# nz0001na/MorphGANformer

Measured on AMD Instinct MI355X. Metric: latent-projection iters/sec @1024^2, k=17 latents, higher is better.
Workload: dtype f32; 1 GPU; configs[1]: single 1024x1024 face per GPU, Wing+LPIPS(squeeze)+MSE literal-mode projection step, noise_mode=random, seeded synthetic weights/targets/landmarks; k=17, z_dim=32, targets_per_gpu=1, parallelism=pair-sharded x1, graph_replay=True, loss_generator_overlap=True, steps_per_forward=32

## Files before the change

include/mgf.h:

```cpp
#ifndef MGF_H_
#define MGF_H_

#include <stdint.h>

#ifdef __cplusplus
extern "C" {
#endif

typedef void* mgf_stream_t;

enum { MGF_OK = 0, MGF_EINVAL = -1, MGF_EUNSUPPORTED = -2, MGF_ELAUNCH = -3, MGF_ETOOBIG = -4 };
enum { MGF_F32 = 0, MGF_F64 = 1, MGF_F16 = 2 };
enum { MGF_FILTER_SEPARABLE = 2 };
enum { MGF_FILTER_LARGE = 4 };
enum { MGF_ACT_LINEAR = 1, MGF_ACT_RELU = 2, MGF_ACT_LRELU = 3, MGF_ACT_TANH = 4, MGF_ACT_SIGMOID = 5,
       MGF_ACT_ELU = 6, MGF_ACT_SELU = 7, MGF_ACT_SOFTPLUS = 8, MGF_ACT_SWISH = 9,
       MGF_ACT_RELU_POST = 10 };

const char* mgf_last_error(void);
int mgf_version(void);
int mgf_device_ok(void);

int mgf_bias_act(void* y, const void* x, const void* b, const void* xref, const void* yref, const void* dy,
                 int dtype, int64_t numel, int64_t step_b, int64_t size_b,
// ... 79 lines not shown
int mgf_conv1x1_force_shape(int32_t channel_blocks);

int mgf_conv3x3s2_few_inputs_f32(float* y, const float* x, const float* w, const float* bias, int32_t n, int32_t cin, int32_t in_h,
                                 int32_t in_w, int32_t cout, int32_t relu, mgf_stream_t stream);
int mgf_tconv3x3s2_few_outputs_f32(float* y, const float* x, const float* wp, int32_t n, int32_t cin, int32_t h, int32_t w, int32_t cout,
                                   int32_t cout_pad, int32_t pitch, int64_t y_plane, int64_t y_batch, mgf_stream_t stream);
int mgf_conv3x3_winograd3_up2res_f32(float* y, const float* x, const float* u, const float* in_scale, const float* out_scale,
                                     const float* residual_low, int32_t n, int32_t cin, int32_t h, int32_t w, int32_t cout,
                                     int32_t out_scale_stride, const mgf_epilogue* ep, mgf_stream_t stream);
int mgf_winograd3_force_shape(int32_t shape);
int mgf_conv3x3_winograd3_rgb_f32(float* rgb_out, const float* x, const float* u, const float* in_scale, const float* out_scale,
                                  const float* rgb_w, const float* rgb_bias, int32_t n, int32_t cin, int32_t h, int32_t w, int32_t cout,
                                  int32_t out_scale_stride, int32_t rgb_channels, mgf_stream_t stream);
int mgf_conv3x3_winograd_f32(float* y, const float* x, const float* u, const float* in_scale, const float* out_scale, int32_t n,
                             int32_t cin, int32_t h, int32_t w, int32_t cout, int32_t out_scale_stride, const mgf_epilogue* ep,
                             mgf_stream_t stream);

int mgf_tconv3x3s2_border_f32(float* t, const float* x, const float* wp, const float* in_scale, const float* out_scale, int32_t n,
                              int32_t cin, int32_t h, int32_t w, int32_t cout, int32_t cout_pad, int64_t t_pitch, int64_t t_plane,
                              int64_t t_batch, int64_t out_scale_stride, mgf_stream_t stream);

int mgf_tconv3x3s2_blur_f32(float* y, const float* x, const float* wp, const float* in_scale, const float* out_scale, const float* f1d,
                            float gain, int32_t n, int32_t cin, int32_t h, int32_t w, int32_t cout, int32_t cout_pad, int64_t y_pitch,
                            int64_t y_plane, int64_t y_batch, int64_t out_scale_stride, const mgf_epilogue* ep, mgf_stream_t stream);

int mgf_tconv3x3s2_winograd_f32(float* t, const float* x, const float* u, const float* in_scale, const float* out_scale, int32_t n,
                                int32_t cin, int32_t h, int32_t w, int32_t cout, int32_t pitch, int64_t t_plane, int64_t t_batch,
                                int64_t out_scale_stride, mgf_stream_t stream);
int mgf_tconv_winograd_weights_f32(float* u, const float* w, int32_t cout, int32_t cin, double gain, mgf_stream_t stream);

int mgf_pack_conv_weights(float* wp, float* wsq, const float* w, int32_t cout, int32_t cin, int32_t kh, int32_t kw,
                          int32_t cout_pad, float gain, int32_t flip, mgf_stream_t stream);

typedef struct mgf_style_job {
    const float* aff_w;
    const float* aff_b;
    const float* wsq;
    float* s;
    float* d;
    int32_t cin, cout;
    int32_t w_offset;
    float aff_gain, style_gain;
} mgf_style_job;
int mgf_demod_f32(float* d, const float* s, const float* wsq, int32_t n, int32_t cin, int32_t cout, mgf_stream_t stream);
int mgf_demod_bwd_f32(float* ds, const float* dd, const float* d, const float* s, const float* wsq, int32_t n, int32_t cin, int32_t cout,
                      mgf_stream_t stream);
int mgf_style_demod(const mgf_style_job* job, const float* ws, int64_t ws_stride_n, int32_t n, int32_t wdim, mgf_stream_t stream);
int mgf_style_demod_multi(const mgf_style_job* jobs_dev, int32_t njobs, const float* ws, int64_t ws_stride_n,
                          int32_t n, int32_t wdim, int32_t max_cin, mgf_stream_t stream);

int mgf_duplex_attention(float* y, const float* x, const float* wqc, const float* spos, const float* vwb,
                         int32_t n, int32_t c, int32_t f, int32_t t,
                         const mgf_epilogue* ep, int32_t ep_w, float* probs, int32_t* argmax, mgf_stream_t stream);

int mgf_att_map_upsample_f32(float* out, const float* probs, int32_t n, int32_t side, int32_t t, int32_t out_res, int32_t layer,
                             int32_t n_layers, mgf_stream_t stream);

typedef struct mgf_attn_job {
    const float* wmv;
    const float* bmv;
    float* vwb;
    int32_t c;
    int32_t w_offset;
} mgf_attn_job;
int mgf_attn_values(const mgf_attn_job* job, const float* ws, int64_t ws_stride_n, int64_t ws_stride_t, int32_t n, int32_t t,
                    int32_t wdim, mgf_stream_t stream);
int mgf_attn_values_multi(const mgf_attn_job* jobs_dev, int32_t njobs, const float* ws, int64_t ws_stride_n, int64_t ws_stride_t,
                          int32_t n, int32_t t, int32_t wdim, mgf_stream_t stream);

int mgf_randn_f32(float* out, int64_t n, uint64_t seed, void* state, mgf_stream_t stream);
int mgf_rgb_weights_f32(float* out, const float* w, const float* s, int32_t n, int32_t c, int32_t cout, mgf_stream_t stream);
int mgf_randn_keyed_f32(float* out, const int32_t* sides, int32_t n_layers, int32_t n, const uint64_t* key, const int32_t* step,
                        int32_t step_stride, int32_t step_add, int32_t step_max, int32_t aux0, int32_t aux_add, mgf_stream_t stream);
int mgf_torgb_compose_weights_f32(float* w_eff, const float* w_last, const float* s_last, const float* d_last, const float* w_rgb,
                                  const float* s_rgb, int32_t n, int32_t cin, int32_t cout, int32_t rgb_channels, mgf_stream_t stream);
int mgf_conv3x3_few_outputs_f32(float* y, const float* x, const float* w, const float* bias, int32_t n, int32_t cin, int32_t h, int32_t wd,
                                int32_t cout, mgf_stream_t stream);

int64_t mgf_mapping_param_floats(int32_t k, int32_t dim, int32_t n_res_layers);
int mgf_mapping_forward(float* w, const float* z, const float* params, int32_t n, int32_t k, int32_t dim,
                        int32_t n_res_layers, int32_t normalize_global, mgf_stream_t stream);

int64_t mgf_reduce_scratch_floats(void);
int mgf_mse_f32(float* out, const float* a, const float* b, int32_t n, int64_t numel, int64_t b_batch_stride, float scale,
                int32_t accumulate, float* scratch, mgf_stream_t stream);
int64_t mgf_dssim_scratch_bytes(int32_t n, int32_t c, int32_t h, int32_t w);
int mgf_dssim_u8_f32(float* out, const float* img, const float* target, int32_t n, int32_t c, int32_t h, int32_t w, int64_t t_batch_stride,
                     float data_range, float scale, int32_t accumulate, void* scratch, mgf_stream_t stream);
int mgf_dssim_f32(float* out, const float* img, const float* target, int32_t n, int32_t c, int32_t h, int32_t w, int64_t t_batch_stride,
                  float data_range, float scale, int32_t accumulate, void* scratch, mgf_stream_t stream);
int mgf_dssim_grad_f32(float* dimg, float* out, const float* img, const float* target, int32_t n, int32_t c, int32_t h, int32_t w,
                       int64_t t_batch_stride, float data_range, float scale, int32_t accumulate_dimg, int32_t accumulate_out, void* scratch,
                       mgf_stream_t stream);
int64_t mgf_msssim_scratch_bytes(int32_t n, int32_t c, int32_t h, int32_t w, int32_t levels);
int mgf_msssim_f32(float* out, const float* img, const float* target, int32_t n, int32_t c, int32_t h, int32_t w, int64_t t_batch_stride,
                   const double* weights, int32_t levels, float data_range, float scale, int32_t accumulate, void* scratch, mgf_stream_t stream);
int mgf_msssim_grad_f32(float* dimg, float* out, const float* img, const float* target, int32_t n, int32_t c, int32_t h, int32_t w,
                        int64_t t_batch_stride, const double* weights, int32_t levels, float data_range, float scale, int32_t accumulate_dimg,
                        int32_t accumulate_out, void* scratch, mgf_stream_t stream);
int64_t mgf_lbp_scratch_bytes(int32_t n);
int mgf_lbp_gray224_u8(uint8_t* gray, const float* img, const int32_t* tables, int32_t n, int32_t h, int32_t w, int32_t true_rgb_order,
                       mgf_stream_t stream);
int mgf_lbp_codes_u8(uint8_t* codes, const uint8_t* gray, const double* offsets, int32_t n, mgf_stream_t stream);
int mgf_lbp_distance_f64(double* out, const uint8_t* gray, const uint8_t* target_codes, const double* offsets, int32_t n, void* scratch,
                         mgf_stream_t stream);
int mgf_wing_loss_f64(double* out, const double* pred, const double* target, int32_t n, int64_t numel, double omega, double epsilon,
// ... 240 lines not shown
```

morphganformer_amd/csrc/attention.hip:

```cpp
#include "mgf_common.h"

namespace {

typedef float v2f __attribute__((ext_vector_type(2)));
__device__ __forceinline__ void att_fma_row(v2f (&s2)[8], float xv, const float4* w4) {
    const v2f x2 = {xv, xv};
#pragma unroll
    for (int q = 0; q < 4; ++q) {
        const float4 w = w4[q];
        const v2f lo = {w.x, w.y}, hi = {w.z, w.w};
        s2[2 * q] += x2 * lo;
        s2[2 * q + 1] += x2 * hi;
    }
}
__device__ __forceinline__ float att_dot_row(const v2f (&s2)[8], const float4* w4) {
    v2f g2 = {0.f, 0.f};
#pragma unroll
    for (int q = 0; q < 4; ++q) {
        const float4 w = w4[q];
        const v2f lo = {w.x, w.y}, hi = {w.z, w.w};
        g2 += s2[2 * q] * lo;
        g2 += s2[2 * q + 1] * hi;
    }
    return g2.x + g2.y;
}

constexpr int TMAX = 16;
constexpr int UNR = 4;

struct AttnParams {
    float* y;
    const float* x;
    const float* wqc;
    const float* spos;
    const float* vwb;
    int n, c, f, t;
    int c_pad;
    mgf_epilogue ep;
    int has_ep;
    float* probs;
    int32_t* argmax;
};

template <int PXB, int NCH>
__global__ __launch_bounds__(256) void duplex_attention_kernel(AttnParams p) {
    constexpr int G = 256 / PXB;
    extern __shared__ float lds[];
    float* tab = lds;
    float* part = lds + (size_t)p.c_pad * TMAX;
    const int tid = threadIdx.x;
    const int px = tid % PXB, grp = tid / PXB;
    const int n = blockIdx.y;
    const int f0 = blockIdx.x * PXB;
    const int f = f0 + px;
    const bool valid = f < p.f;
    const int fc = valid ? f : p.f - 1;
    const float* xn = p.x + (int64_t)n * p.c * p.f;
    const int T = p.t;

    float xreg[NCH > 0 ? NCH : 1];
    if (NCH > 0) {
#pragma unroll
        for (int k = 0; k < NCH; ++k) {
            const int c = (k / UNR) * G * UNR + grp * UNR + (k % UNR);
            xreg[k] = xn[(int64_t)c * p.f + fc];
        }
    }

    auto stage_table = [&](const float* src) {
        if (T == TMAX) {
            const int n4 = p.c * (TMAX / 4), n4_pad = p.c_pad * (TMAX / 4);
            const float4* s4 = reinterpret_cast<const float4*>(src);
            float4* d4 = reinterpret_cast<float4*>(tab);
            for (int i0 = tid; i0 < n4_pad; i0 += 256 * 4) {
                float4 v[4];
#pragma unroll
                for (int u = 0; u < 4; ++u) {
                    const int i = i0 + 256 * u;
                    v[u] = i < n4 ? s4[i] : make_float4(0.f, 0.f, 0.f, 0.f);
                }
#pragma unroll
                for (int u = 0; u < 4; ++u) {
                    const int i = i0 + 256 * u;
                    if (i < n4_pad) d4[i] = v[u];
                }
            }
        } else {
            for (int i = tid; i < p.c_pad * TMAX; i += 256) {
                const int c = i / TMAX, t = i % TMAX;
                tab[i] = (c < p.c && t < T) ? src[(int64_t)c * T + t] : 0.f;
            }
        }
    };
    stage_table(p.wqc);
// ... 333 lines not shown
            for (int g = 0; g < G; ++g) v += part[(g * (TMAX + 1) + t) * PXB + px];
            fin[t * PXB + px] = v;
        }
        __syncthreads();
        float m = -3.0e38f;
#pragma unroll
        for (int t = 0; t < TMAX; ++t) {
            const float v = fin[t * PXB + px] + spk[t];
            m = fmaxf(m, v);
            s[t] = v;
        }
        sq = fin[TMAX * PXB + px];
        float den = 0.f;
        int best = 0;
        float bestv = -3.0e38f;
#pragma unroll
        for (int t = 0; t < TMAX; ++t) {
            if (s[t] > bestv) { bestv = s[t]; best = t; }
            s[t] = __expf(s[t] - m);
            den += s[t];
        }
        const float inv = 1.f / den;
        const float rs = rsqrtf(sq / (float)p.c + 1e-8f);
#pragma unroll
        for (int t = 0; t < TMAX; ++t) s[t] *= inv;
        if (grp == 0 && valid) {
            if (p.probs)
                for (int t = 0; t < TMAX; ++t) p.probs[((int64_t)n * p.f + f) * TMAX + t] = s[t];
            if (p.argmax) p.argmax[(int64_t)n * p.f + f] = best;
        }
#pragma unroll
        for (int q = 0; q < TMAX / 2; ++q) s2[q] = v2f{s[2 * q] * rs, s[2 * q + 1] * rs};

        float* yn = p.y + (int64_t)n * p.c * p.f;
#pragma unroll
        for (int k = 0; k < NCH; ++k) {
            const int c = (k / UNR) * G * UNR + grp * UNR + (k % UNR);
            const float g = att_dot_row(s2, reinterpret_cast<const float4*>(tabv + c * TMAX));
            float v = xk[k] * g;
            if (p.has_ep) {
                v += nzk;
                if (p.ep.bias) v += p.ep.bias[c];
                if (p.ep.act == MGF_ACT_LRELU) v = v > 0.f ? v : v * p.ep.alpha;
                else if (p.ep.act == MGF_ACT_RELU) v = v > 0.f ? v : 0.f;
                v *= p.ep.gain;
                v += rk[k];
            }
            if (valid) yn[(int64_t)c * p.f + f] = v;
        }
    }
}

typedef float f32x16 __attribute__((ext_vector_type(16)));
template <int NW>
__global__ __launch_bounds__(NW * 64, NW == 4 ? 4 : 2) void duplex_attention_mfma_kernel(AttnParams p) {
    __shared__ float red[NW][9][64];
    const int tid = threadIdx.x, lane = tid & 63;
    const int wv = __builtin_amdgcn_readfirstlane(tid >> 6);
    const int l31 = lane & 31, half = lane >> 5;
    const int n = blockIdx.y, f0 = blockIdx.x * 32;
    const int cw0 = wv * 64;
    const int64_t nb = (int64_t)n * p.c * p.f;
    const bool ep = p.has_ep != 0;
    const __amdgpu_buffer_rsrc_t rx = __builtin_amdgcn_make_buffer_rsrc((void*)(p.x + nb), 0, p.c * p.f * 4, 0x00020000);
    const float* resp = (ep && p.ep.residual) ? p.ep.residual + nb : nullptr;
    const __amdgpu_buffer_rsrc_t rres = __builtin_amdgcn_make_buffer_rsrc((void*)(resp ? resp : p.x), 0, resp ? p.c * p.f * 4 : 0, 0x00020000);
    const __amdgpu_buffer_rsrc_t rq = __builtin_amdgcn_make_buffer_rsrc((void*)p.wqc, 0, p.c * TMAX * 4, 0x00020000);
    const __amdgpu_buffer_rsrc_t rv = __builtin_amdgcn_make_buffer_rsrc((void*)(p.vwb + (int64_t)n * p.c * TMAX), 0, p.c * TMAX * 4, 0x00020000);
    const __amdgpu_buffer_rsrc_t rsp = __builtin_amdgcn_make_buffer_rsrc((void*)p.spos, 0, p.f * TMAX * 4, 0x00020000);
    const float* biasp = (ep && p.ep.bias) ? p.ep.bias : nullptr;
    const __amdgpu_buffer_rsrc_t rb = __builtin_amdgcn_make_buffer_rsrc((void*)(biasp ? biasp : p.x), 0, biasp ? p.c * 4 : 0, 0x00020000);
    auto rowof = [](int r) { return (r & 3) + 8 * (r >> 2); };

    const unsigned xo = (unsigned)((cw0 + 4 * half) * p.f + f0 + l31) * 4u;
    const unsigned qo = l31 < TMAX ? (unsigned)((cw0 + 4 * half) * TMAX + l31) * 4u : 0xFFFFFFF0u;
    float xr[2][16], a1[2][16];
#pragma unroll
    for (int cb = 0; cb < 2; ++cb)
#pragma unroll
        for (int r = 0; r < 16; ++r) {
            const int ch = 32 * cb + rowof(r);
            xr[cb][r] = __builtin_bit_cast(float, __builtin_amdgcn_raw_buffer_load_b32(rx, xo, ch * p.f * 4, 0));
            a1[cb][r] = __builtin_bit_cast(float, __builtin_amdgcn_raw_buffer_load_b32(rq, qo, ch * TMAX * 4, 0));
        }
    float sp[8];
#pragma unroll
    for (int r = 0; r < 8; ++r)
        sp[r] = __builtin_bit_cast(float, __builtin_amdgcn_raw_buffer_load_b32(rsp, (unsigned)((f0 + l31) * TMAX + 4 * half) * 4u, rowof(r) * 4, 0));
    float nz = 0.f;
    if (ep && p.ep.noise) nz = p.ep.noise[(int64_t)(p.ep.noise_n > 1 ? n : 0) * p.f + f0 + l31] * (p.ep.noise_strength ? *p.ep.noise_strength : 1.f);

    f32x16 acc;
#pragma unroll
    for (int r = 0; r < 16; ++r) acc[r] = 0.f;
    float sq = 0.f;
#pragma unroll
    for (int cb = 0; cb < 2; ++cb)
#pragma unroll
        for (int r = 0; r < 16; ++r) {
            acc = __builtin_amdgcn_mfma_f32_32x32x2f32(a1[cb][r], xr[cb][r], acc, 0, 0, 0);
            sq += xr[cb][r] * xr[cb][r];
        }
    float rr[2][16];
#pragma unroll
    for (int cb = 0; cb < 2; ++cb)
#pragma unroll
        for (int r = 0; r < 16; ++r)
            rr[cb][r] = __builtin_bit_cast(float, __builtin_amdgcn_raw_buffer_load_b32(rres, xo, (32 * cb + rowof(r)) * p.f * 4, 0));
#pragma unroll
    for (int r = 0; r < 8; ++r) red[wv][r][lane] = acc[r];
    red[wv][8][lane] = sq;
    __syncthreads();
    float s[8];
#pragma unroll
    for (int r = 0; r < 8; ++r) {
        float v = sp[r];
#pragma unroll
        for (int w = 0; w < NW; ++w) v += red[w][r][lane];
        s[r] = v;
    }
    sq = 0.f;
#pragma unroll
    for (int w = 0; w < NW; ++w) sq += red[w][8][lane];
    sq += __shfl_xor(sq, 32, 64);
    float m = s[0];
    int best = 4 * half;
#pragma unroll
    for (int r = 1; r < 8; ++r) {
        if (s[r] > m) { m = s[r]; best = rowof(r) + 4 * half; }
    }
    {
        const float om = __shfl_xor(m, 32, 64);
        const int ob = __shfl_xor(best, 32, 64);
        if (om > m || (om == m && ob < best)) { m = om; best = ob; }
    }
    float den = 0.f;
#pragma unroll
    for (int r = 0; r < 8; ++r) { s[r] = __expf(s[r] - m); den += s[r]; }
    den += __shfl_xor(den, 32, 64);
    const float inv = 1.f / den;
    const float rs = rsqrtf(sq / (float)p.c + 1e-8f);
    if (wv == 0) {
        if (p.probs) {
#pragma unroll
            for (int r = 0; r < 8; ++r) p.probs[((int64_t)n * p.f + f0 + l31) * TMAX + rowof(r) + 4 * half] = s[r] * inv;
        }
        if (p.argmax && half == 0) p.argmax[(int64_t)n * p.f + f0 + l31] = best;
    }
    const float ps = inv * rs;
#pragma unroll
    for (int r = 0; r < 8; ++r) s[r] *= ps;

    float* yn = p.y + nb;
    const float slope = !ep ? 1.f : (p.ep.act == MGF_ACT_LRELU ? p.ep.alpha : (p.ep.act == MGF_ACT_RELU ? 0.f : 1.f));
    const float gain = ep ? p.ep.gain : 1.f;
#pragma unroll
    for (int cb = 0; cb < 2; ++cb) {
        const unsigned vo = (unsigned)((cw0 + 32 * cb + l31) * TMAX + 4 * half) * 4u;
        const float4 va = __builtin_bit_cast(float4, __builtin_amdgcn_raw_buffer_load_b128(rv, vo, 0, 0));
        const float4 vb = __builtin_bit_cast(float4, __builtin_amdgcn_raw_buffer_load_b128(rv, vo + 32u, 0, 0));
        float bv[16];
#pragma unroll
        for (int r = 0; r < 16; ++r)
            bv[r] = __builtin_bit_cast(float, __builtin_amdgcn_raw_buffer_load_b32(rb, (unsigned)(cw0 + 32 * cb + 4 * half) * 4u, rowof(r) * 4, 0));
        const float a2[8] = {va.x, va.y, va.z, va.w, vb.x, vb.y, vb.z, vb.w};
        f32x16 g;
#pragma unroll
        for (int r = 0; r < 16; ++r) g[r] = 0.f;
#pragma unroll
        for (int j = 0; j < 8; ++j) g = __builtin_amdgcn_mfma_f32_32x32x2f32(a2[j], s[j], g, 0, 0, 0);
#pragma unroll
        for (int r = 0; r < 16; ++r) {
            float v = xr[cb][r] * g[r];
            v += nz;
            v += bv[r];
            v = v > 0.f ? v : v * slope;
            v = v * gain + rr[cb][r];
            yn[(int64_t)(cw0 + 32 * cb + rowof(r) + 4 * half) * p.f + f0 + l31] = v;
        }
    }
}

__global__ __launch_bounds__(256) void att_map_upsample_kernel(float* out, const float* probs, int t, int s, int R, int layer, int layers,
                                                               int64_t total) {
    const int f = R / s;
    for (int64_t i = (int64_t)blockIdx.x * 256 + threadIdx.x; i < total; i += (int64_t)gridDim.x * 256) {
        const int x = (int)(i % R);
        int64_t r = i / R;
        const int y = (int)(r % R);
        r /= R;
        const int tt = (int)(r % t);
        const int64_t n = r / t;
        out[(((n * t + tt) * layers + layer) * R + y) * (int64_t)R + x] = probs[(n * s * s + (int64_t)(y / f) * s + x / f) * t + tt];
    }
}

template <int PXB>
void launch_attention(const AttnParams& p, size_t lds, hipStream_t st) {
    constexpr int G = 256 / PXB;
    const int nch = (p.c % (G * UNR) == 0) ? p.c / G : 0;
    if (p.t == TMAX && (nch == 16 || nch == 32 || nch == 64) && (nch * G) % 64 == 0) {
        const size_t lds_r = ((size_t)p.c * TMAX + (size_t)(G + 1) * (TMAX + 1) * PXB) * sizeof(float);
        static const char* nb_env = mgf_knob("MGF_ATTN_NBLK");
        constexpr int NBLK = 4;
        if (PXB == 16 && nch == 16 && p.f >= 4096 && p.f % (PXB * NBLK) == 0 && !(nb_env && nb_env[0] == '1')) {
            const size_t lds_2 = ((size_t)2 * p.c * TMAX + (size_t)(G + 1) * (TMAX + 1) * PXB) * sizeof(float);
            hipLaunchKernelGGL((duplex_attention_blocks_kernel<PXB, 16, NBLK>), dim3((unsigned)(p.f / (PXB * NBLK)), p.n), dim3(256), lds_2, st, p);
            return;
        }
        const dim3 grid((unsigned)mgf_cdiv(p.f, PXB), p.n);
        if (nch == 16) hipLaunchKernelGGL((duplex_attention_reg_kernel<PXB, 16>), grid, dim3(256), lds_r, st, p);
        else if (nch == 32) hipLaunchKernelGGL((duplex_attention_reg_kernel<PXB, 32>), grid, dim3(256), lds_r, st, p);
        else hipLaunchKernelGGL((duplex_attention_reg_kernel<PXB, 64>), grid, dim3(256), lds_r, st, p);
        return;
    }
    const dim3 grid((unsigned)mgf_cdiv(p.f, PXB), p.n);
    hipLaunchKernelGGL((duplex_attention_kernel<PXB, 0>), grid, dim3(256), lds, st, p);
}

}

extern "C" int mgf_duplex_attention(float* y, const float* x, const float* wqc, const float* spos, const float* vwb, int32_t n,
                                    int32_t c, int32_t f, int32_t t, const mgf_epilogue* ep, int32_t ep_w, float* probs,
                                    int32_t* argmax, mgf_stream_t stream) {
    (void)ep_w;
    MGF_REQUIRE(y && x && wqc && spos && vwb, MGF_EINVAL, "duplex_attention: null pointer");
    MGF_REQUIRE(n >= 1 && c >= 1 && f >= 1, MGF_EINVAL, "duplex_attention: bad shape");
    MGF_REQUIRE(t >= 1 && t <= TMAX, MGF_EUNSUPPORTED, "duplex_attention: supports 1..%d latent components (got %d)", TMAX, t);
    MGF_REQUIRE(n <= 65535 && (int64_t)n * c * f <= INT32_MAX, MGF_ETOOBIG, "duplex_attention: tensor too large");
    if (ep) MGF_REQUIRE(ep->act == 0 || ep->act == MGF_ACT_LINEAR || ep->act == MGF_ACT_LRELU || ep->act == MGF_ACT_RELU,
                        MGF_EUNSUPPORTED, "duplex_attention: epilogue activation %d unsupported", ep->act);
    AttnParams p;
    p.y = y; p.x = x; p.wqc = wqc; p.spos = spos; p.vwb = vwb; p.n = n; p.c = c; p.f = f; p.t = t;
    p.has_ep = ep != nullptr; p.probs = probs; p.argmax = argmax;
    if (ep) { p.ep = *ep; if (p.ep.act == 0) p.ep.act = MGF_ACT_LINEAR; } else { p.ep = mgf_epilogue{}; p.ep.gain = 1.f; }
    MGF_REQUIRE(((uintptr_t)wqc % 16 == 0) && ((uintptr_t)vwb % 16 == 0), MGF_EINVAL, "duplex_attention: tables must be 16-byte aligned");
    static const char* mf_env = mgf_knob("MGF_ATTN_MFMA");
    if (t == TMAX && (c == 256 || c == 512) && f % 32 == 0 && !(mf_env && mf_env[0] == '0')) {
        hipStream_t st0 = (hipStream_t)stream;
        if (c == 256) hipLaunchKernelGGL((duplex_attention_mfma_kernel<4>), dim3((unsigned)(f / 32), n), dim3(256), 0, st0, p);
        else hipLaunchKernelGGL((duplex_attention_mfma_kernel<8>), dim3((unsigned)(f / 32), n), dim3(512), 0, st0, p);
        MGF_CHECK_LAUNCH("duplex_attention");
        return MGF_OK;
    }
    static const char* pxb_env = mgf_knob("MGF_ATTN_PXB");
    const int pxb = pxb_env ? atoi(pxb_env) : (f > 16384 ? 64 : 16);
    const int g = 256 / pxb;
    p.c_pad = (int)(mgf_cdiv(c, UNR * g) * UNR * g);
    const size_t lds = ((size_t)p.c_pad * TMAX + (size_t)g * (TMAX + 1) * pxb) * sizeof(float);
    MGF_REQUIRE(lds <= 64 * 1024, MGF_EUNSUPPORTED, "duplex_attention: %d channels need %zu bytes of LDS (> 64 KiB)", c, lds);
    hipStream_t st = (hipStream_t)stream;
    if (pxb == 64) launch_attention<64>(p, lds, st);
    else if (pxb == 32) launch_attention<32>(p, lds, st);
    else launch_attention<16>(p, lds, st);
    MGF_CHECK_LAUNCH("duplex_attention");
    return MGF_OK;
}

extern "C" int mgf_att_map_upsample_f32(float* out, const float* probs, int32_t n, int32_t side, int32_t t, int32_t out_res, int32_t layer,
                                        int32_t n_layers, mgf_stream_t stream) {
    MGF_REQUIRE(out && probs && n >= 1 && side >= 1 && t >= 1 && n_layers >= 1, MGF_EINVAL, "att_map_upsample: bad arguments");
    MGF_REQUIRE(layer >= 0 && layer < n_layers, MGF_EINVAL, "att_map_upsample: layer %d outside 0..%d", layer, n_layers - 1);
    MGF_REQUIRE(out_res >= side && out_res % side == 0, MGF_EINVAL, "att_map_upsample: the image resolution %d must be a multiple of the map side %d", out_res, side);
    const int64_t total = (int64_t)n * t * out_res * out_res;
    hipLaunchKernelGGL(att_map_upsample_kernel, dim3(mgf_stream_grid(total, 256, 4)), dim3(256), 0, (hipStream_t)stream, out, probs, t, side,
                       out_res, layer, n_layers, total);
    MGF_CHECK_LAUNCH("att_map_upsample");
    return MGF_OK;
}
```

morphganformer_amd/engine.py:

```python
from __future__ import annotations

import ctypes as C
import math
import os
from dataclasses import dataclass, field

import numpy as np
import torch

from . import _lib
from . import conv as cv
from .synth_weights import GeneratorConfig

SQRT2 = math.sqrt(2.0)
SQRT_HALF = math.sqrt(0.5)
USE_WINOGRAD = os.environ.get("MGF_WINOGRAD", "1") != "0"
WINOGRAD_MAX_RES = int(os.environ.get("MGF_WINOGRAD_MAX_RES", "1024"))
TCONV_WINO_MAX_RES = int(os.environ.get("MGF_TCONV_WINO_MAX_RES", "256"))
BF_DIRECT_MAX_RES = int(os.environ.get("MGF_BF_DIRECT_MAX_RES", "128"))
MAX_LOCAL_LATENTS = 16
LATENT_WIDTH = 32


def check_supported(cfg: GeneratorConfig) -> None:
# ... 198 lines not shown
        self._ws_cache = {}
        self.taps = None
        self.fuse_torgb = True
        self.skip_fused = {}
        self.fuse_skip_up = os.environ.get("MGF_FUSE_SKIP_UP", "1") != "0"
        self.last_noise = ("none", None)
        self.side = torch.cuda.Stream(device=self.device)
        self.overlap_skip = os.environ.get("MGF_OVERLAP_SKIP", "0") != "0"
        self.torgb_compose = os.environ.get("MGF_TORGB_COMPOSE", "1") != "0"
        self._workspaces, self._pins = {}, {}
        self.noise_seed, self._noise_epoch = int(torch.initial_seed()) & 0xFFFFFFFFFFFFFFFF, None
        self.noise_state = torch.zeros(2, dtype=torch.int64, device=self.device)
        self._keyed_words = {}
        self._alloc(max_batch)

    _WS_FIELDS = ("n", "lean", "w_buf", "styles", "demods", "vtabs", "noise_rand", "bufs", "img", "const_in", "rgbw", "w_eff", "style_jobs", "n_style_jobs",
                  "max_style_cin", "attn_jobs", "n_attn_jobs", "style_jobs_pl", "attn_jobs_pl", "ws_bytes", "ws_gen")

    def _alloc(self, n, lean=None):
        cur = (getattr(self, "n", None), getattr(self, "lean", False))
        lean = cur[1] if lean is None else bool(lean)
        if cur[0] is not None and cur in self._workspaces:
            self._workspaces[cur]["noise_rand"] = self.noise_rand
        key = (n, lean)
        ws = self._workspaces.pop(key, None)
        if ws is None:
            self._evict_for(n, lean)
            self._create(n, lean)
            ws = {k: getattr(self, k) for k in self._WS_FIELDS}
        self._workspaces[key] = ws
        for k, v in ws.items():
            setattr(self, k, v)

    def pin(self, key=None):
        key = (self.n, self.lean) if key is None else key
        self._pins[key] = self._pins.get(key, 0) + 1
        return key

    def unpin(self, key):
        if self._pins.get(key, 0) > 0:
            self._pins[key] -= 1

    def _evict_for(self, n, lean):
        budget = float(os.environ.get("MGF_WORKSPACE_GB", "160")) * 2 ** 30
        need = self._workspace_bytes(n, lean)
        total = sum(w["ws_bytes"] for w in self._workspaces.values())
        cur = (getattr(self, "n", None), getattr(self, "lean", False))
        for m in list(self._workspaces):
            if total + need <= budget:
                break
            if self._pins.get(m, 0) == 0 and m != cur:
                total -= self._workspaces.pop(m)["ws_bytes"]

    def _fuses_skip_up(self, l1, n):
        res = l1.res
        if l1.pcb is not None and res <= BF_DIRECT_MAX_RES:
            return False
        return bool(self.fuse_skip_up and self.plan.fir_is_1331 and cv.WINOGRAD_FORM == 3 and l1.attn is None and res % 2 == 0
                    and cv.conv3x3_takes_winograd(l1.conv, n, res, res) and l1.conv.u.ndim == 4)

    def _lean_arenas(self, n):
        cfg = self.cfg
        conv1 = {lp.res: lp for lp in self.plan.layers if lp.name.endswith(".conv1")}
        a = dict(T=0, U=0, V=0, W0=0, W1=0, S=0, SL=0)
        for i, res in enumerate(cfg.block_resolutions):
            c, px = cfg.channels(res), res * res
            a["U"] = max(a["U"], c * px)
            a["W%d" % (i & 1)] = max(a["W%d" % (i & 1)], c * px)
            if res > 4:
                a["T"] = max(a["T"], c * (res + 1) * cv.tconv_pitch(res // 2, self.tpitch_align))
                a["SL"] = max(a["SL"], c * px // 4)
                if not self._fuses_skip_up(conv1[res], n):
                    a["S"] = max(a["S"], c * px)
                if cfg.has_attention(res):
                    a["V"] = max(a["V"], c * px)
            if res == cfg.img_resolution:
                a["T"] = max(a["T"], c * px)
        return a

    def _workspace_bytes(self, n, lean=False):
        cfg = self.cfg
        if lean:
            return 4 * n * (sum(self._lean_arenas(n).values()) + cfg.img_channels * cfg.img_resolution ** 2)
        per = 0
        for res in cfg.block_resolutions:
            c = cfg.channels(res)
            planes = 1 + (4 if res > 4 else 0) + (1 if res > 4 and cfg.has_attention(res) else 0) + (1 if cfg.has_attention(res) else 0) \
                + (1 if res == cfg.img_resolution else 0)
            per += planes * c * res * res
        return 4 * n * (per + cfg.img_channels * cfg.img_resolution ** 2)

    def _create(self, n, lean=False):
        cfg, dev, P = self.cfg, self.device, self.plan
        e = lambda *s: torch.empty(s, dtype=torch.float32, device=dev)
        self.n, self.lean = n, bool(lean)
        self._gen_counter = getattr(self, "_gen_counter", 0) + 1
        self.ws_gen = self._gen_counter
        self.w_buf = e(n, cfg.k, cfg.w_dim)
        self.styles = e(n, P.s_total)
        self.demods = e(n, P.d_total)
        self.vtabs = e(n, max(P.v_total, 1))
        self.noise_rand = None
        self.bufs = {}
        if lean:
            arena = {k: e(n * v) for k, v in self._lean_arenas(n).items() if v}
            conv1 = {lp.res: lp for lp in P.layers if lp.name.endswith(".conv1")}
            view = lambda k, *shape: arena[k][:int(np.prod(shape))].view(*shape)
            for i, res in enumerate(cfg.block_resolutions):
                c, att, W = cfg.channels(res), cfg.has_attention(res), "W%d" % (i & 1)
                b = {"conv1": view("U" if att else W, n, c, res, res)}
                if att:
                    b["conv1a"] = view(W, n, c, res, res)
                if res > 4:
                    b["skip_low"] = view("SL", n, c, res // 2, res // 2)
                    b["t"] = view("T", n, c, res + 1, cv.tconv_pitch(res // 2, self.tpitch_align))
                    b["conv0"] = view("U", n, c, res, res)
                    if att:
                        b["conv0a"] = view("V", n, c, res, res)
                    if not self._fuses_skip_up(conv1[res], n):
                        b["skip"] = view("S", n, c, res, res)
                if res == cfg.img_resolution:
                    b["last"] = view("T", n, c, res, res)
                self.bufs[res] = b
        for res in ([] if lean else cfg.block_resolutions):
            c = cfg.channels(res)
            b = {"conv1": e(n, c, res, res)}
            if res > 4:
                b["skip_low"] = e(n, c, res // 2, res // 2)
                b["skip"] = e(n, c, res, res)
                b["t"] = e(n, c, res + 1, cv.tconv_pitch(res // 2, self.tpitch_align))
                b["conv0"] = e(n, c, res, res)
                if cfg.has_attention(res):
                    b["conv0a"] = e(n, c, res, res)
            if cfg.has_attention(res):
                b["conv1a"] = e(n, c, res, res)
            if res == cfg.img_resolution:
                b["last"] = e(n, c, res, res)
            self.bufs[res] = b
        self.img = e(n, cfg.img_channels, cfg.img_resolution, cfg.img_resolution)
        self.const_in = P.const.unsqueeze(0).repeat(n, 1, 1, 1).contiguous()
        self.rgbw = e(n, cfg.img_channels, cfg.channels(cfg.img_resolution))
        self.w_eff = e(n, cfg.img_channels, cfg.channels(cfg.img_resolution), 3, 3)
        self.ws_bytes = self._workspace_bytes(n, lean)
        self._build_jobs(n)

    def _build_jobs(self, n):
        cfg, P = self.cfg, self.plan
        D, NW = cfg.w_dim, cfg.num_ws

        def tables(per_layer):
            sj = (_lib.StyleJob * len(P.layers))()
            aj = []
            for i, lp in enumerate(P.layers):
                g_off = ((cfg.k - 1) * NW + lp.slot) * D if per_layer else (cfg.k - 1) * D
                sj[i] = _lib.StyleJob(lp.aff_w.data_ptr(), lp.aff_b.data_ptr(), _lib.ptr(lp.packed.wsq) if lp.demod else 0,
                                      self.styles.data_ptr() + 4 * lp.s_off * n,
                                      (self.demods.data_ptr() + 4 * lp.d_off * n) if lp.demod else 0,
                                      lp.cin, lp.cout, g_off, 1.0 / math.sqrt(D), lp.style_gain)
                if lp.attn is not None:
                    aj.append(_lib.AttnJob(lp.attn.wmv.data_ptr(), lp.attn.bmv.data_ptr(),
                                           self.vtabs.data_ptr() + 4 * lp.attn.v_off * n, lp.attn.c, lp.slot * D if per_layer else 0))
            sjt = _lib.device_table(sj, self.device)
            ajt = _lib.device_table((_lib.AttnJob * len(aj))(*aj), self.device) if aj else None
            return sjt, ajt, len(aj)

        self.style_jobs, self.attn_jobs, self.n_attn_jobs = tables(False)
        self.style_jobs_pl, self.attn_jobs_pl, _ = tables(True)
        self.n_style_jobs = len(P.layers)
        self.max_style_cin = max(lp.cin for lp in P.layers)

    def _s(self, lp):
        return self.styles.view(-1)[lp.s_off * self.n:(lp.s_off + lp.cin) * self.n].view(self.n, lp.cin)
# ... 217 lines not shown
    def _noise_views(self, n, sizes):
        out, off = {}, 0
        for name, r in sizes:
            out[name] = self.noise_rand[off * n:(off + r * r) * n].view(n, r * r)
            off += r * r
        return out

    def _keyed_word(self, value, dtype, what):
        if isinstance(value, torch.Tensor):
            _lib.require_gpu(value)
            if value.dtype != dtype or value.numel() < 1 or not value.is_contiguous():
                raise _lib.MgfError(f"noise_mode='keyed': {what} must be a contiguous device {dtype} tensor (got {value.dtype}, {tuple(value.shape)})")
            return value
        if value is None:
            raise _lib.MgfError(f"noise_mode='keyed' needs {what} (a device {dtype} tensor or an int): the maps are a function of noise_key and "
                                "noise_step, there is no stream to continue")
        v = int(value)
        if dtype == torch.int64:
            v &= 0xFFFFFFFFFFFFFFFF
            v -= (v >> 63) << 64
        t = self._keyed_words.get((dtype, v))
        if t is None:
            if torch.cuda.is_current_stream_capturing():
                raise _lib.MgfError(f"noise_mode='keyed': {what} is a host int inside a graph capture; pass a device tensor")
            if len(self._keyed_words) >= 256:
                self._keyed_words.clear()
            t = self._keyed_words[(dtype, v)] = torch.tensor([v], dtype=dtype, device=self.device)
        return t

    def _draw_noise_keyed(self, n, key, step, step_stride=0, step_add=1, step_max=None, aux=(1, 0)):
        sizes = self._noise_buffer(n)
        key_t = self._keyed_word(key, torch.int64, "noise_key")
        step_t = self._keyed_word(step, torch.int32, "noise_step")
        step_stride, step_add = int(step_stride), int(step_add)
        if step_stride < 0 or (n - 1) * step_stride >= step_t.numel():
            raise _lib.MgfError(f"noise_mode='keyed': noise_step holds {step_t.numel()} counter(s), {n} samples at stride {step_stride} read past them")
        step_max = 2 ** 31 - 1 if step_max is None else int(step_max)
        sides = (C.c_int32 * len(sizes))(*[r for _, r in sizes])
        _lib.check(_lib.lib().mgf_randn_keyed_f32(self.noise_rand.data_ptr(), sides, len(sizes), n, key_t.data_ptr(), step_t.data_ptr(), step_stride,
                                                  step_add, step_max, int(aux[0]), int(aux[1]), _lib.stream_ptr()), "randn_keyed")
        return self._noise_views(n, sizes)

    def _bf_direct(self, lp, n, residual_low):
        return (lp.pcb is not None and lp.kind == "conv3" and residual_low is None and 32 <= lp.res <= BF_DIRECT_MAX_RES
                and n * (lp.res // 8) * (lp.res // 32) * (lp.cout // 32) >= 512)

    def _layer(self, lp, x, B, key, noise_mode, noises, residual, residual_low=None):
        n = x.shape[0]
        noise, noise_n = self._noise_for(lp, noise_mode, noises)
        ep = _lib.make_epilogue(bias=lp.bias, noise=noise, noise_strength=lp.noise_strength if noise is not None else None,
                                noise_n=noise_n, act="lrelu", alpha=0.2, gain=lp.act_gain, residual=residual)
        has_att = lp.attn is not None
        s, d = self._s(lp), self._d(lp)
        if (lp.kind == "tconv" and not has_att and self.taps is None and lp.pcb is None
                and cv.tconv_blur_ok(n, x.shape[1], x.shape[2], x.shape[3], lp.cout, B[key], self.plan.fir1, ep)
                and not (lp.wino_t is not None and cv.tconv_winograd_ok(n, x.shape[1], x.shape[2], x.shape[3], lp.cout, B["t"]))):
            y = cv.tconv3x3s2_blur_forward(x, lp.pc, self.plan.fir1, 4.0, in_scale=s, out_scale=d, epilogue=ep, out=B[key], t=B["t"],
                                           f2d=self.plan.fir, wt=lp.wino_t)
        elif lp.kind == "tconv":
            t = cv.tconv3x3s2_forward(x, lp.pc, in_scale=s, out_scale=d, out=B["t"], bf=lp.pcb, wt=lp.wino_t)
            y = cv.upfirdn_into(B[key], t, self.plan.fir, up=1, pad=(1, 1, 1, 1), gain=4.0, epilogue=None if has_att else ep,
                                separable=True)
        elif self._bf_direct(lp, n, residual_low):
            y = cv.conv_forward(x, lp.conv.pc, pad=(1, 1), in_scale=s, out_scale=d, epilogue=None if has_att else ep, out=B[key], bf=lp.pcb)
        else:
            y = cv.conv3x3_forward(x, lp.conv, in_scale=s, out_scale=d, epilogue=None if has_att else ep, out=B[key], residual_low=residual_low)
        if self.taps is not None:
            self.taps[lp.name + ":conv"] = y
        if has_att:
            a = lp.attn
            out = B[key + "a"]
            probs = argmax = None
            if self.att_maps is not None:
                probs = torch.empty([n, a.f, self.cfg.k - 1], dtype=torch.float32, device=self.device)
                argmax = torch.empty([n, a.f], dtype=torch.int32, device=self.device)
                self.att_maps[lp.name] = (probs, argmax)
            rc = _lib.lib().mgf_duplex_attention(out.data_ptr(), y.data_ptr(), a.wqc.data_ptr(), a.spos.data_ptr(),
                                                 self._v(lp).data_ptr(), n, a.c, a.f, self.cfg.k - 1, C.byref(ep), lp.res,
                                                 _lib.ptr(probs), _lib.ptr(argmax), _lib.stream_ptr())
            _lib.check(rc, "duplex_attention")
            y = out
        return y

    def forward_workspace(self, z=None, c=None, ws=None, truncation_psi=1, truncation_cutoff=None, return_img=True, return_att=False,
                          return_ws=False, subnet=None, noise_mode="random", noises=None, fused_modconv=None, att_format="tensor", lean=False,
                          noise_key=None, noise_step=None, noise_step_stride=0, noise_step_add=1, noise_step_max=None, noise_aux=(1, 0)):
        if noise_mode == "keyed" and (noise_key is None or noise_step is None):
            raise _lib.MgfError("Generator: noise_mode='keyed' needs noise_key and noise_step (the maps are a function of the two)")
        lean = bool(lean) and self.taps is None and not return_att
        nb = (z if ws is None else ws)
        if nb is not None and (nb.shape[0], lean) != (self.n, self.lean):
            self._alloc(nb.shape[0], lean)
        return_tensor = False
        if subnet is not None:
            return_ws, return_img, return_att, return_tensor = subnet == "mapping", subnet == "synthesis", False, True
        if att_format not in ("tensor", "maps"):
            raise ValueError(f"att_format must be 'tensor' or 'maps' (got {att_format!r})")
        ws_out = None
        if ws is None:
            if z is None:
                raise _lib.MgfError("Generator: pass z or ws")
            w = self._mapping_into(z)
            if truncation_psi != 1 and truncation_cutoff is not None:
                w_in = ws_out = self._truncate(w, truncation_psi, truncation_cutoff).contiguous()
            else:
                w_in = self.w_avg.lerp(w, truncation_psi) if truncation_psi != 1 else w
        else:
            _lib.require_gpu(ws)
            if ws.ndim != 4 or tuple(ws.shape[1:]) != (self.cfg.k, self.num_ws, self.cfg.w_dim):
                raise _lib.MgfError(f"Generator: ws must be [n, {self.cfg.k}, {self.num_ws}, {self.cfg.w_dim}] (got {tuple(ws.shape)})")
            if ws.shape[0] != self.n:
                self._alloc(ws.shape[0])
            w_in = ws_out = ws.contiguous().float()
        ret = ()
        if return_img or return_att:
            img = self.synthesis(w_in if w_in.ndim == 4 else w_in.contiguous(), noise_mode=noise_mode, noises=noises, return_att=return_att,
                                 noise_key=noise_key, noise_step=noise_step, noise_step_stride=noise_step_stride, noise_step_add=noise_step_add,
                                 noise_step_max=noise_step_max, noise_aux=noise_aux)
            if return_img:
                ret += (img,)
            if return_att:
                ret += (self.att_maps if att_format == "maps" else self.list2tensor(self.att_maps),)
        if return_ws:
            ret += (ws_out if ws_out is not None else w_in.unsqueeze(2).expand(-1, -1, self.num_ws, -1),)
        return ret[0] if return_tensor else ret

    def __call__(self, *args, **kwargs):
        ret = self.forward_workspace(*args, **kwargs)
        own = lambda t: t.clone() if isinstance(t, torch.Tensor) else t
        return own(ret) if not isinstance(ret, tuple) else tuple(own(t) for t in ret)
```

Before: 790.5 iters/s.

## Fuse 2x skip upsampling into the MFMA attention epilogue for attention layers

Adds a variant of the MFMA duplex-attention kernel that reads the half-resolution skip residual directly and applies the [1,3,3,1] bilinear upsample inline (9/16, 3/16, 1/16 weights) in the epilogue. Loads are software-pipelined in groups of eight. The engine now allows skip-upsample fusion for attention layers, so it no longer has to materialise the full-resolution skip buffer or run a separate upsample pass. The costs are extra gathered loads per output and more register pressure in the kernel. The fused path only covers c=256/512 with 16 latents and even square maps.

After: 788.6 iters/s. No clear change (-0.2%).

```diff
diff --git a/include/mgf.h b/include/mgf.h
--- a/include/mgf.h
+++ b/include/mgf.h
@@ -155,6 +155,9 @@
 int mgf_duplex_attention(float* y, const float* x, const float* wqc, const float* spos, const float* vwb,
                          int32_t n, int32_t c, int32_t f, int32_t t,
                          const mgf_epilogue* ep, int32_t ep_w, float* probs, int32_t* argmax, mgf_stream_t stream);
+int mgf_duplex_attention_up2res(float* y, const float* x, const float* wqc, const float* spos, const float* vwb, const float* residual_low,
+                                int32_t n, int32_t c, int32_t f, int32_t t, const mgf_epilogue* ep, int32_t ep_w, float* probs,
+                                int32_t* argmax, mgf_stream_t stream);
 
 int mgf_att_map_upsample_f32(float* out, const float* probs, int32_t n, int32_t side, int32_t t, int32_t out_res, int32_t layer,
                              int32_t n_layers, mgf_stream_t stream);
diff --git a/morphganformer_amd/csrc/attention.hip b/morphganformer_amd/csrc/attention.hip
--- a/morphganformer_amd/csrc/attention.hip
+++ b/morphganformer_amd/csrc/attention.hip
@@ -40,6 +40,8 @@
     int has_ep;
     float* probs;
     int32_t* argmax;
+    const float* residual_low;
+    int res;
 };
 
 template <int PXB, int NCH>
@@ -479,7 +481,7 @@
 }
 
 typedef float f32x16 __attribute__((ext_vector_type(16)));
-template <int NW>
+template <int NW, bool LOW>
 __global__ __launch_bounds__(NW * 64, NW == 4 ? 4 : 2) void duplex_attention_mfma_kernel(AttnParams p) {
     __shared__ float red[NW][9][64];
     const int tid = threadIdx.x, lane = tid & 63;
@@ -529,11 +531,49 @@
             sq += xr[cb][r] * xr[cb][r];
         }
     float rr[2][16];
-#pragma unroll
-    for (int cb = 0; cb < 2; ++cb)
-#pragma unroll
-        for (int r = 0; r < 16; ++r)
-            rr[cb][r] = __builtin_bit_cast(float, __builtin_amdgcn_raw_buffer_load_b32(rres, xo, (32 * cb + rowof(r)) * p.f * 4, 0));
+    constexpr int LG = 8;
+    float lowq[LG][4];
+    unsigned lo4[4] = {0u, 0u, 0u, 0u};
+    int hh4 = 0;
+    __amdgpu_buffer_rsrc_t rlow = rres;
+    auto low_request = [&](int g) {
+#pragma unroll
+        for (int u = 0; u < LG; ++u) {
+            const int k = LG * g + u;
+            const int so = (32 * (k >> 4) + rowof(k & 15)) * hh4;
+#pragma unroll
+            for (int q = 0; q < 4; ++q) lowq[u][q] = __builtin_bit_cast(float, __builtin_amdgcn_raw_buffer_load_b32(rlow, lo4[q], so, 0));
+        }
+    };
+    auto low_mix = [&](int g) {
+#pragma unroll
+        for (int u = 0; u < LG; ++u) {
+            const int k = LG * g + u;
+            rr[k >> 4][k & 15] = 0.5625f * lowq[u][0] + 0.1875f * (lowq[u][1] + lowq[u][2]) + 0.0625f * lowq[u][3];
+        }
+    };
+    if (LOW) {
+        const int hs = p.res >> 1, f = f0 + l31;
+        const int oy = f / p.res, ox = f - oy * p.res;
+        const int my = oy >> 1, mx = ox >> 1;
+        const int ny = my + ((oy & 1) ? 1 : -1), nx = mx + ((ox & 1) ? 1 : -1);
+        const bool vy = (unsigned)ny < (unsigned)hs, vx = (unsigned)nx < (unsigned)hs;
+        hh4 = hs * hs * 4;
+        rlow = __builtin_amdgcn_make_buffer_rsrc((void*)(p.residual_low + (int64_t)n * p.c * hs * hs), 0, p.c * hh4, 0x00020000);
+        const unsigned cbase = (unsigned)((cw0 + 4 * half) * hs * hs);
+        const unsigned out = 0xFFFFFFF0u;
+        lo4[0] = (cbase + (unsigned)(my * hs + mx)) * 4u;
+        lo4[1] = vx ? (cbase + (unsigned)(my * hs + nx)) * 4u : out;
+        lo4[2] = vy ? (cbase + (unsigned)(ny * hs + mx)) * 4u : out;
+        lo4[3] = (vx && vy) ? (cbase + (unsigned)(ny * hs + nx)) * 4u : out;
+        low_request(0);
+    } else {
+#pragma unroll
+        for (int cb = 0; cb < 2; ++cb)
+#pragma unroll
+            for (int r = 0; r < 16; ++r)
+                rr[cb][r] = __builtin_bit_cast(float, __builtin_amdgcn_raw_buffer_load_b32(rres, xo, (32 * cb + rowof(r)) * p.f * 4, 0));
+    }
 #pragma unroll
     for (int r = 0; r < 8; ++r) red[wv][r][lane] = acc[r];
     red[wv][8][lane] = sq;
@@ -589,7 +629,7 @@
         float bv[16];
 #pragma unroll
         for (int r = 0; r < 16; ++r)
-            bv[r] = __builtin_bit_cast(float, __builtin_amdgcn_raw_buffer_load_b32(rb, (unsigned)(cw0 + 32 * cb + 4 * half) * 4u, rowof(r) * 4, 0));
+            if (!LOW) bv[r] = __builtin_bit_cast(float, __builtin_amdgcn_raw_buffer_load_b32(rb, (unsigned)(cw0 + 32 * cb + 4 * half) * 4u, rowof(r) * 4, 0));
         const float a2[8] = {va.x, va.y, va.z, va.w, vb.x, vb.y, vb.z, vb.w};
         f32x16 g;
 #pragma unroll
@@ -598,9 +638,14 @@
         for (int j = 0; j < 8; ++j) g = __builtin_amdgcn_mfma_f32_32x32x2f32(a2[j], s[j], g, 0, 0, 0);
 #pragma unroll
         for (int r = 0; r < 16; ++r) {
+            if (LOW && (16 * cb + r) % LG == 0) {
+                const int lg = (16 * cb + r) / LG;
+                low_mix(lg);
+                if (lg + 1 < 32 / LG) low_request(lg + 1);
+            }
             float v = xr[cb][r] * g[r];
             v += nz;
-            v += bv[r];
+            v += LOW ? __builtin_bit_cast(float, __builtin_amdgcn_raw_buffer_load_b32(rb, (unsigned)(cw0 + 32 * cb + 4 * half) * 4u, rowof(r) * 4, 0)) : bv[r];
             v = v > 0.f ? v : v * slope;
             v = v * gain + rr[cb][r];
             yn[(int64_t)(cw0 + 32 * cb + rowof(r) + 4 * half) * p.f + f0 + l31] = v;
@@ -659,14 +704,14 @@
                         MGF_EUNSUPPORTED, "duplex_attention: epilogue activation %d unsupported", ep->act);
     AttnParams p;
     p.y = y; p.x = x; p.wqc = wqc; p.spos = spos; p.vwb = vwb; p.n = n; p.c = c; p.f = f; p.t = t;
-    p.has_ep = ep != nullptr; p.probs = probs; p.argmax = argmax;
+    p.has_ep = ep != nullptr; p.probs = probs; p.argmax = argmax; p.residual_low = nullptr; p.res = 0;
     if (ep) { p.ep = *ep; if (p.ep.act == 0) p.ep.act = MGF_ACT_LINEAR; } else { p.ep = mgf_epilogue{}; p.ep.gain = 1.f; }
     MGF_REQUIRE(((uintptr_t)wqc % 16 == 0) && ((uintptr_t)vwb % 16 == 0), MGF_EINVAL, "duplex_attention: tables must be 16-byte aligned");
     static const char* mf_env = mgf_knob("MGF_ATTN_MFMA");
     if (t == TMAX && (c == 256 || c == 512) && f % 32 == 0 && !(mf_env && mf_env[0] == '0')) {
         hipStream_t st0 = (hipStream_t)stream;
-        if (c == 256) hipLaunchKernelGGL((duplex_attention_mfma_kernel<4>), dim3((unsigned)(f / 32), n), dim3(256), 0, st0, p);
-        else hipLaunchKernelGGL((duplex_attention_mfma_kernel<8>), dim3((unsigned)(f / 32), n), dim3(512), 0, st0, p);
+        if (c == 256) hipLaunchKernelGGL((duplex_attention_mfma_kernel<4, false>), dim3((unsigned)(f / 32), n), dim3(256), 0, st0, p);
+        else hipLaunchKernelGGL((duplex_attention_mfma_kernel<8, false>), dim3((unsigned)(f / 32), n), dim3(512), 0, st0, p);
         MGF_CHECK_LAUNCH("duplex_attention");
         return MGF_OK;
     }
@@ -684,6 +729,33 @@
     return MGF_OK;
 }
 
+extern "C" int mgf_duplex_attention_up2res(float* y, const float* x, const float* wqc, const float* spos, const float* vwb,
+                                           const float* residual_low, int32_t n, int32_t c, int32_t f, int32_t t, const mgf_epilogue* ep,
+                                           int32_t ep_w, float* probs, int32_t* argmax, mgf_stream_t stream) {
+    const int32_t res = ep_w;
+    MGF_REQUIRE(y && x && wqc && spos && vwb && residual_low, MGF_EINVAL, "duplex_attention_up2res: null pointer");
+    MGF_REQUIRE(n >= 1 && c >= 1 && f >= 1 && res >= 1, MGF_EINVAL, "duplex_attention_up2res: bad shape");
+    MGF_REQUIRE(n <= 65535 && (int64_t)n * c * f <= INT32_MAX, MGF_ETOOBIG, "duplex_attention_up2res: tensor too large");
+    MGF_REQUIRE(!ep || !ep->residual, MGF_EUNSUPPORTED, "duplex_attention_up2res: the residual comes at full OR at half resolution");
+    MGF_REQUIRE(res % 2 == 0 && (int64_t)res * res == f, MGF_EUNSUPPORTED,
+                "duplex_attention_up2res: needs a square map with an even side (res %d, f %d)", res, f);
+    MGF_REQUIRE(t == TMAX && (c == 256 || c == 512) && f % 32 == 0, MGF_EUNSUPPORTED,
+                "duplex_attention_up2res: only the MFMA form takes the half-resolution residual (c = 256 or 512, 16 latents, f %% 32 == 0; "
+                "got c %d, t %d, f %d)", c, t, f);
+    if (ep) MGF_REQUIRE(ep->act == 0 || ep->act == MGF_ACT_LINEAR || ep->act == MGF_ACT_LRELU || ep->act == MGF_ACT_RELU,
+                        MGF_EUNSUPPORTED, "duplex_attention_up2res: epilogue activation %d unsupported", ep->act);
+    MGF_REQUIRE(((uintptr_t)wqc % 16 == 0) && ((uintptr_t)vwb % 16 == 0), MGF_EINVAL, "duplex_attention_up2res: tables must be 16-byte aligned");
+    AttnParams p;
+    p.y = y; p.x = x; p.wqc = wqc; p.spos = spos; p.vwb = vwb; p.n = n; p.c = c; p.f = f; p.t = t; p.c_pad = c;
+    p.has_ep = 1; p.probs = probs; p.argmax = argmax; p.residual_low = residual_low; p.res = res;
+    if (ep) { p.ep = *ep; if (p.ep.act == 0) p.ep.act = MGF_ACT_LINEAR; } else { p.ep = mgf_epilogue{}; p.ep.gain = 1.f; p.ep.act = MGF_ACT_LINEAR; }
+    hipStream_t st = (hipStream_t)stream;
+    if (c == 256) hipLaunchKernelGGL((duplex_attention_mfma_kernel<4, true>), dim3((unsigned)(f / 32), n), dim3(256), 0, st, p);
+    else hipLaunchKernelGGL((duplex_attention_mfma_kernel<8, true>), dim3((unsigned)(f / 32), n), dim3(512), 0, st, p);
+    MGF_CHECK_LAUNCH("duplex_attention_up2res");
+    return MGF_OK;
+}
+
 extern "C" int mgf_att_map_upsample_f32(float* out, const float* probs, int32_t n, int32_t side, int32_t t, int32_t out_res, int32_t layer,
                                         int32_t n_layers, mgf_stream_t stream) {
     MGF_REQUIRE(out && probs && n >= 1 && side >= 1 && t >= 1 && n_layers >= 1, MGF_EINVAL, "att_map_upsample: bad arguments");
diff --git a/morphganformer_amd/engine.py b/morphganformer_amd/engine.py
--- a/morphganformer_amd/engine.py
+++ b/morphganformer_amd/engine.py
@@ -274,12 +274,19 @@
             if self._pins.get(m, 0) == 0 and m != cur:
                 total -= self._workspaces.pop(m)["ws_bytes"]
 
-    def _fuses_skip_up(self, l1, n):
+    def _fuses_skip_up(self, l1, n, layout=False):
         res = l1.res
+        if not (self.fuse_skip_up and self.plan.fir_is_1331 and res % 2 == 0):
+            return False
+        if l1.attn is not None:
+            a = l1.attn
+            mfma = (self.cfg.k - 1 == 16 and a.c in (256, 512) and a.f % 32 == 0 and a.f == res * res and n <= 65535
+                    and n * a.c * a.f <= 2 ** 31 - 1 and os.environ.get("MGF_ATTN_MFMA", "1")[:1] != "0")
+            free = self.fuse_torgb and (layout or self.taps is None)
+            return bool(mfma and free)
         if l1.pcb is not None and res <= BF_DIRECT_MAX_RES:
             return False
-        return bool(self.fuse_skip_up and self.plan.fir_is_1331 and cv.WINOGRAD_FORM == 3 and l1.attn is None and res % 2 == 0
-                    and cv.conv3x3_takes_winograd(l1.conv, n, res, res) and l1.conv.u.ndim == 4)
+        return bool(cv.WINOGRAD_FORM == 3 and cv.conv3x3_takes_winograd(l1.conv, n, res, res) and l1.conv.u.ndim == 4)
 
     def _lean_arenas(self, n):
         cfg = self.cfg
@@ -292,7 +299,7 @@
             if res > 4:
                 a["T"] = max(a["T"], c * (res + 1) * cv.tconv_pitch(res // 2, self.tpitch_align))
                 a["SL"] = max(a["SL"], c * px // 4)
-                if not self._fuses_skip_up(conv1[res], n):
+                if not self._fuses_skip_up(conv1[res], n, layout=True):
                     a["S"] = max(a["S"], c * px)
                 if cfg.has_attention(res):
                     a["V"] = max(a["V"], c * px)
@@ -339,7 +346,7 @@
                     b["conv0"] = view("U", n, c, res, res)
                     if att:
                         b["conv0a"] = view("V", n, c, res, res)
-                    if not self._fuses_skip_up(conv1[res], n):
+                    if not self._fuses_skip_up(conv1[res], n, layout=True):
                         b["skip"] = view("S", n, c, res, res)
                 if res == cfg.img_resolution:
                     b["last"] = view("T", n, c, res, res)
@@ -663,6 +670,7 @@
                                 noise_n=noise_n, act="lrelu", alpha=0.2, gain=lp.act_gain, residual=residual)
         has_att = lp.attn is not None
         s, d = self._s(lp), self._d(lp)
+        conv_low = None if has_att else residual_low
         if (lp.kind == "tconv" and not has_att and self.taps is None and lp.pcb is None
                 and cv.tconv_blur_ok(n, x.shape[1], x.shape[2], x.shape[3], lp.cout, B[key], self.plan.fir1, ep)
                 and not (lp.wino_t is not None and cv.tconv_winograd_ok(n, x.shape[1], x.shape[2], x.shape[3], lp.cout, B["t"]))):
@@ -672,10 +680,10 @@
             t = cv.tconv3x3s2_forward(x, lp.pc, in_scale=s, out_scale=d, out=B["t"], bf=lp.pcb, wt=lp.wino_t)
             y = cv.upfirdn_into(B[key], t, self.plan.fir, up=1, pad=(1, 1, 1, 1), gain=4.0, epilogue=None if has_att else ep,
                                 separable=True)
-        elif self._bf_direct(lp, n, residual_low):
+        elif self._bf_direct(lp, n, conv_low):
             y = cv.conv_forward(x, lp.conv.pc, pad=(1, 1), in_scale=s, out_scale=d, epilogue=None if has_att else ep, out=B[key], bf=lp.pcb)
         else:
-            y = cv.conv3x3_forward(x, lp.conv, in_scale=s, out_scale=d, epilogue=None if has_att else ep, out=B[key], residual_low=residual_low)
+            y = cv.conv3x3_forward(x, lp.conv, in_scale=s, out_scale=d, epilogue=None if has_att else ep, out=B[key], residual_low=conv_low)
         if self.taps is not None:
             self.taps[lp.name + ":conv"] = y
         if has_att:
@@ -686,9 +694,15 @@
                 probs = torch.empty([n, a.f, self.cfg.k - 1], dtype=torch.float32, device=self.device)
                 argmax = torch.empty([n, a.f], dtype=torch.int32, device=self.device)
                 self.att_maps[lp.name] = (probs, argmax)
-            rc = _lib.lib().mgf_duplex_attention(out.data_ptr(), y.data_ptr(), a.wqc.data_ptr(), a.spos.data_ptr(),
-                                                 self._v(lp).data_ptr(), n, a.c, a.f, self.cfg.k - 1, C.byref(ep), lp.res,
-                                                 _lib.ptr(probs), _lib.ptr(argmax), _lib.stream_ptr())
+            if residual_low is not None:
+                assert residual_low.is_contiguous() and tuple(residual_low.shape) == (n, a.c, lp.res // 2, lp.res // 2)
+                rc = _lib.lib().mgf_duplex_attention_up2res(out.data_ptr(), y.data_ptr(), a.wqc.data_ptr(), a.spos.data_ptr(),
+                                                            self._v(lp).data_ptr(), residual_low.data_ptr(), n, a.c, a.f, self.cfg.k - 1,
+                                                            C.byref(ep), lp.res, _lib.ptr(probs), _lib.ptr(argmax), _lib.stream_ptr())
+            else:
+                rc = _lib.lib().mgf_duplex_attention(out.data_ptr(), y.data_ptr(), a.wqc.data_ptr(), a.spos.data_ptr(),
+                                                     self._v(lp).data_ptr(), n, a.c, a.f, self.cfg.k - 1, C.byref(ep), lp.res,
+                                                     _lib.ptr(probs), _lib.ptr(argmax), _lib.stream_ptr())
             _lib.check(rc, "duplex_attention")
             y = out
         return y
```
